# topopt/TopOpt_in_PETSc

Measured on AMD Instinct MI355X. Metric: DOF-updates/s per design iter (assembly+PCG+filter), higher is better.
Workload: dtype f64; 1 GPU; cantilever128: cantilever 128x128x128 elements (6440067 DOF), z-slabs over 1 GPU(s), rmin=2.56h density filter, CG + 5-level GMG (Chebyshev(2)-Jacobi, coarse exact (banded Cholesky + explicit triangular inverse per assembly), Galerkin, cycles per level 1,3,1,1), rtol 1e-05, fine-level eig element bound, cold start, filtered synthetic density seed 12345; n_dof=6440067, levels=5, cycles=1,3,1,1, coarse_solve=direct (2187 rows), cg_its=11, parallelism=zslab1, comm=none, comm_ranks=1, halo_overlap=0

## Files before the change

### include/topopt_amd.h

```cpp
#ifndef TOPOPT_AMD_H
#define TOPOPT_AMD_H

#include <stddef.h>
#include <stdint.h>

#ifdef __cplusplus
extern "C" {
#endif

#define TP_OK 0
#define TP_ERR_ARG 1
#define TP_ERR_STATE 2
#define TP_ERR_DIVERGED 3
#define TP_ERR_COMM 4
#define TP_ERR_HIP 1000

#define TP_MAX_LEVELS 10

typedef struct tp_comm {
    void *user;
    double *send_lo, *send_hi, *recv_lo, *recv_hi;
    double *red;
    long cap;
    int (*exchange)(void *user, long n);
// ... 124 lines not shown
double tp_elasticity_level_lambda(const tp_elasticity *e, int level);
double tp_elasticity_level_lambda_min(const tp_elasticity *e, int level);
int tp_elasticity_coarse_direct_active(const tp_elasticity *e);
int tp_xcd_status(int *giveups, int *xcd_forms_off, int *defer_off);
int tp_elasticity_level_apply(tp_elasticity *e, int level, const double *u, double *y);
int tp_elasticity_level_diag(tp_elasticity *e, int level, double *d);
int tp_elasticity_precond(tp_elasticity *e, const double *r, double *z);
int tp_elasticity_level_pc(tp_elasticity *e, int level, int pc, const double *r, double *z);
int tp_elasticity_level_gmres(tp_elasticity *e, int level, int pc, int m, int its, double rtol, const double *b, double *x,
                              int zero_guess, int *its_done);
int tp_elasticity_smooth(tp_elasticity *e, int level, const double *b, double *x, int k, int zero_guess);
int tp_elasticity_smooth_dot(tp_elasticity *e, int level, const double *b, double *x, int k, int zero_guess, double *dot);
int tp_elasticity_level_residual(tp_elasticity *e, int level, const double *b, const double *x, double *r);
int tp_elasticity_restrict(tp_elasticity *e, int level, const double *rf, double *rc);
int tp_elasticity_prolong_add(tp_elasticity *e, int level, const double *xc, double *xf);
int tp_elasticity_last_stats(const tp_elasticity *e, double *alg_bytes, double *flops, long *kernel_launches);
int tp_elasticity_last_op_form(const tp_elasticity *e, int *form4);

typedef struct tp_filter tp_filter;
int tp_filter_create(tp_filter **f, tp_grid *g, int filterType, double rmin, const tp_solver_opts *pde_opts);
int tp_filter_mult_h(tp_filter *f, const double *x, double *y);
int tp_filter_destroy(tp_filter *f);
int tp_filter_stencil_width(const tp_filter *f);
int tp_filter_last_kernel(const tp_filter *f);
int tp_filter_get_hs(tp_filter *f, double *Hs);
int tp_filter_get_kf(const tp_filter *f, double *kf_host_64);
int tp_filter_project(tp_filter *f, const double *x, double *xTilde, double *xPhys, int projectionFilter, double beta,
                      double eta);
int tp_filter_gradients(tp_filter *f, const double *x, const double *xTilde, double *dfdx, int m, double **dgdx,
                        int projectionFilter, double beta, double eta);
// ... 69 lines not shown
```

### topopt_in_petsc_amd/api.py

```python
import ctypes as C
import os
from dataclasses import dataclass

import torch

from . import lib as _lib
from .comm import SlabComm
from .partition import SlabPartition


class TopOptError(RuntimeError):
    def __init__(self, code, where):
        names = {1: "TP_ERR_ARG", 2: "TP_ERR_STATE", 3: "TP_ERR_DIVERGED", 4: "TP_ERR_COMM"}
        msg = names.get(code, "hipError %d" % (code - 1000) if code >= 1000 else str(code))
        super().__init__("%s failed: %s" % (where, msg))
        self.code = code


def _chk(code, where):
    if code != 0:
        raise TopOptError(code, where)


def check_body_force(b, x_low):
# ... 556 lines not shown

    def level_residual(self, l, b, x):
        r = torch.zeros_like(x)
        _chk(self.L.tp_elasticity_level_residual(self.handle, l, _ptr(b), _ptr(x), _ptr(r)), "tp_elasticity_level_residual")
        return r

    def restrict(self, l, rf):
        rc = self.level_vec(l + 1)
        _chk(self.L.tp_elasticity_restrict(self.handle, l, _ptr(rf), _ptr(rc)), "tp_elasticity_restrict")
        return rc

    def prolong_add(self, l, xc, xf):
        _chk(self.L.tp_elasticity_prolong_add(self.handle, l, _ptr(xc), _ptr(xf)), "tp_elasticity_prolong_add")
        return xf

    def pop_stats(self):
        b, f, n = C.c_double(), C.c_double(), C.c_long()
        self.L.tp_elasticity_last_stats(self.handle, C.byref(b), C.byref(f), C.byref(n))
        return b.value, f.value, n.value

    def last_op_form(self):
        f = (C.c_int * 4)()
        _chk(self.L.tp_elasticity_last_op_form(self.handle, f), "tp_elasticity_last_op_form")
        return tuple(f)


class Filter:

    def __init__(self, grid, filterType, rmin, pde_opts=None):
        self.grid, self.L = grid, grid.L
# ... 282 lines not shown
```

### topopt_in_petsc_amd/csrc/mg.h

```cpp
#pragma once
#include <algorithm>
#include <thread>

#include "galerkin.h"
#include "grid.h"
#include "operators.h"
#include "coarse_run.h"
#include "matfree_tile.h"
#include "fine_tile.h"
#include "fine_u4.h"
#include "coarse_direct.h"
#include "mg_kernels.h"

enum { LV_MATFREE = 0, LV_DIA = 1, LV_MACRO = 2 };

template <int DOF>
struct Level {
    Geom g;
    int kind;
    const double *KE;
    const double *E;
    const uint8_t *mask;
    double *S;
    double *Kel;
// ... 118 lines not shown
        long nown = 0;
        int nb = 0;
        int n_bnd = 0;
        bool out_halo = false;
        bool split = false;
        double bytes = 0.0, flops = 0.0;
    };
    template <int EPI>
    int op(int l, NodeArgs a, bool out_halo = false);
    template <int EPI>
    int op_fine(OpLaunch &c, const NodeArgs &a);
    template <int EPI>
    int op_macro(OpLaunch &c, const NodeArgs &a);
    template <int EPI>
    int op_matfree_node(OpLaunch &c, const NodeArgs &a);
    template <int EPI>
    int op_stencil(OpLaunch &c, const NodeArgs &a);
    static void tile_ranges(const Level<DOF> &L, bool split, int pass, int &lo, int &hi, int &r1lo, int &r1hi);
    int after_boundary(int l, double *out);
    static TileArgs tile_args(const Level<DOF> &L, int lo, int hi, int kz, int r1lo, int r1hi);
    static bool three_term(const Level<DOF> &L) { return DOF == 3 && L.kind == LV_MATFREE && L.use_tile; }
    static int fine_generation(const Level<DOF> &L);
    static bool runs_fine_tile(const Level<DOF> &L) { return fine_generation(L) == 2; }
    int drain_halo(int l);
    int drain_halos();
    template <class F>
    int planes_split(int l, double *out, F launch);
    int halo(int l, double *v);
    int apply(int l, double *u, double *y);
    int apply_krylov(double *u, double *y);
// ... 21 lines not shown
    bool xcd_gaveup();
    void xcd_reset_controls();
    void join_side_streams();
    static int run_rows_per_thread(long rows, int *wgs);
    static int xcd_rows_per_thread(long rows, int *wgs);
    int coarse_run_mode(int l, int nsteps) const;
    bool xcd_eligible(int l, long stage_cap, int max_r) const;
    int coarse_run(int l, const double *b, int it0, int k, double sigma, double delta, int mode);

    int alloc_levels();
    void free_levels();
    int setup_matfree_level(int l, const double *h_KE);
    int gather_owned(Level<DOF> &L, const double *src, Level<DOF> &R, double *dst, int nseg, long src_stride = 0,
                     long dst_stride = 0);
    int setup_replicated();
    int smooth(int l, const double *b, int k, bool zero_guess, int dot_slot = -1, bool first_done = false);
    void cheb_window(int l, double *theta, double *delta) const;
    bool can_fuse_rz() const;
    int vcycle_head(const double *b);
    int vcycle(int l, const double *b, int dot_slot = -1, bool first_done = false, bool zero_guess = true);
    int precond(const double *r, double **z, int dot_slot = -1);
    int solve(const double *b, double *x, int *its_out, double *rnorm_out, double *bnorm_out, double *hist, int hist_cap);
};

#include "mg_op.h"
#include "mg_spectra.h"
#include "mg_coarse.h"
#include "mg_cycle.h"
```

### topopt_in_petsc_amd/csrc/mg_cycle.h

```cpp
#pragma once

template <int DOF>
int MGSolver<DOF>::alloc_levels() {
    for (int l = 0; l < nlv; l++) {
        Level<DOF> &L = lv[l];
        L.g = make_geom(grid, l);
        size_t nb = sizeof(double) * (size_t)L.ndof();
        for (double **p : {&L.b, &L.x, &L.x2, &L.r, &L.d, &L.dinv}) {
            TP_HIP(hipMalloc((void **)p, nb));
            TP_HIP(hipMemsetAsync(*p, 0, nb, grid->stream));
        }
    }
    for (int i = nlv; i < LV_SLOTS; i++) {
        lv[i] = Level<DOF>();
        lv[i].b = lv[i].x = lv[i].x2 = lv[i].r = lv[i].d = lv[i].dinv = lv[i].S = lv[i].Kel = nullptr;
    }
    const bool no_rep = sw_no_replicate();
    replicate = allow_replicate && grid->has_comm && nlv > 1 && !no_rep;
    rep0 = nlv - 1;
    if (replicate) {
        const int from_env = sw_replicate_from();
        if (from_env >= 2 && from_env <= nlv - 1) {
            rep0 = from_env;
            while (rep0 < nlv - 1) {
// ... 142 lines not shown
    if (!replicate) return TP_OK;
    for (int l = rep0; l < nlv; l++) {
        Level<DOF> &L = lv[l], &R = lv[rix(l)];
        if (L.kind != LV_DIA) return TP_ERR_STATE;
        TP_TRY(gather_owned(L, L.S, R, R.S, 27 * DOF, L.ndof(), R.ndof()));
        TP_TRY(gather_owned(L, L.dinv, R, R.dinv, 1));
        if constexpr (DOF == 3) {
            TP_LAUNCH(k_dia_sym_fix, dim3((int)((R.g.owned_nodes() + BLK - 1) / BLK)), dim3(BLK), 0, grid->stream, R.g, R.S, (long)R.ndof());
            count_launch(grid);
        }
    }
    return TP_OK;
}

template <int DOF>
int MGSolver<DOF>::smooth(int l, const double *b, int k, bool zero_guess, int dot_slot, bool first_done) {
    if (replicate && l == nlv - 1) {
        Level<DOF> &R = lv[rix(l)];
        TP_TRY(gather_owned(lv[l], b, R, R.b, 1));
        TP_TRY(smooth(rix(l), R.b, k, zero_guess));
        Level<DOF> &L = lv[l];
        TP_HIP(hipMemcpyAsync(L.x, R.x + (long)DOF * L.g.plane() * L.g.gz0, sizeof(double) * (size_t)L.ndof(),
                              hipMemcpyDeviceToDevice, grid->stream));
        return TP_OK;
    }
    Level<DOF> &L = lv[l];
    if (cd.factored && l == cd.level && dot_slot < 0) return coarse_direct_apply(l, b);
    double theta, delta;
    cheb_window(l, &theta, &delta);
    if (!sg_capturing && dot_slot < 0 && k >= 8 && L.kind == LV_DIA && (L.no_comm || !grid->has_comm) && sw_smooth_graph())
        return smooth_replay(l, b, k, zero_guess, first_done, theta, delta);
// ... 15 lines not shown
    if (it >= 1 && dot_slot < 0) {
        const int mode = coarse_run_mode(l, k - it);
        if (mode) return coarse_run(l, b, it, k, sigma, delta, mode);
    }
    for (; it < k; it++) {
        NodeArgs a{};
        a.x = L.x;
        a.out = L.x2;
        a.b = b;
        a.d = L.d;
        a.dinv = L.dinv;
        a.prev_zero = (zero_guess && it == 1) ? 1 : 0;
        if (it == 0) {
            a.c1 = 0.0;
            a.c2 = 1.0 / theta;
        } else {
            const double rn = 1.0 / (2.0 * sigma - rho);
            a.c1 = rn * rho;
            a.c2 = 2.0 * rn / delta;
            rho = rn;
        }
        TP_TRY(halo(l, L.x));
        if (dot_slot >= 0 && it == k - 1) {
            a.partials = grid->partials;
            a.ticket = tail_ticket(grid);
            a.red_out = grid->scal + dot_slot;
            TP_TRY(op<EPI_CHEB_DOT>(l, a));
        } else {
            TP_TRY(op<EPI_CHEB>(l, a, true));
        }
        std::swap(L.x, L.x2);
    }
    return TP_OK;
}

template <int DOF>
void MGSolver<DOF>::cheb_window(int l, double *theta, double *delta) const {
    const Level<DOF> &L = lv[l];
    const bool solve_level = coarsest(l) && base(l) > 0;
    const double lmin = solve_level ? L.lam_min : opt.cheb_lo * L.lam, lmax = opt.cheb_hi * L.lam;
    *theta = 0.5 * (lmax + lmin);
    *delta = 0.5 * (lmax - lmin);
}

template <int DOF>
bool MGSolver<DOF>::can_fuse_rz() const {
    const int fine_v = sw_fine_v();
    const bool off = sw_no_fuse_rz();
// ... 43 lines not shown
    else TP_TRY(restrict_planes(C.g.own_lo, C.g.own_hi - C.g.own_lo + 1));
    count_launch(grid, 8.0 * DOF * (L.g.owned_nodes() + C.g.owned_nodes()), 2.0 * 27 * DOF * C.g.owned_nodes());
    if (enter_rep) {
        const int r = rix(l + 1);
        Level<DOF> &R = lv[r];
        TP_TRY(gather_owned(C, C.b, R, R.b, 1));
        TP_TRY(vcycle(r, R.b, -1, false));
        for (int c = 1; c < cyc; c++) TP_TRY(vcycle(r, R.b, -1, false, false));
        TP_HIP(hipMemcpyAsync(C.x, R.x + (long)DOF * C.g.plane() * C.g.gz0, sizeof(double) * (size_t)C.ndof(),
                              hipMemcpyDeviceToDevice, grid->stream));
    } else {
        TP_TRY(vcycle(l + 1, C.b, -1, fuse_first));
        for (int c = 1; c < cyc; c++) TP_TRY(vcycle(l + 1, C.b, -1, false, false));
        TP_TRY(halo(l + 1, C.x));
    }
    TP_TRY(planes_split(l, L.x, [&](int p0, int np) -> int {
        const long fpl = L.g.plane();
        TP_LAUNCH((k_prolong_add<DOF>), dim3((int)((fpl * np + BLK - 1) / BLK)), dim3(BLK), 0, grid->stream, C.g, L.g, C.x,
                  L.x, fpl * (p0 - L.g.own_lo), fpl * np);
        return TP_OK;
    }));
    count_launch(grid, 8.0 * DOF * (2 * L.g.owned_nodes() + C.g.owned_nodes()), 2.0 * 8 * DOF * L.g.owned_nodes());
    return smooth(l, b, opt.nsmooth, false, l == 0 ? dot_slot : -1);
}

template <int DOF>
int MGSolver<DOF>::precond(const double *r, double **z, int dot_slot) {
    if (opt.ksp_mode == 1) return refksp_precond(*this, r, z);
    TP_TRY(vcycle(0, r, dot_slot));
    TP_TRY(drain_halos());
// ... 156 lines not shown
```

### topopt_in_petsc_amd/csrc/mg_op.h

```cpp
#pragma once

inline int fine_kz(int planes, int tiles, int fine_v, int SLOTS = 768) {
    if (fine_v >= 2 || fine_v == 0) {
        const int tz1 = SLOTS / tiles;
        if (tz1 >= 1) {
            const int kz1 = (planes + tz1 - 1) / tz1;
            const int n1 = tiles * ((planes + kz1 - 1) / kz1);
            if (kz1 >= 3 && kz1 <= 20 && 10 * n1 >= 9 * SLOTS) return kz1;
        }
    }
    int kz = (int)((long)planes * tiles / 5120);
    kz = kz < 8 ? 8 : (kz > 32 ? 32 : kz);
    if ((long)tiles * ((planes + 7) / 8) < SLOTS) kz = (int)((long)planes * tiles / SLOTS);
    const int kmin = (long)tiles * ((planes + 3) / 4) < 256 ? 2 : 4;
    if (kz < kmin) kz = kmin;
    return kz > planes ? planes : kz;
}

template <int DOF>
int MGSolver<DOF>::fine_generation(const Level<DOF> &L) {
    if (!(DOF == 3 && L.kind == LV_MATFREE && L.use_tile)) return 0;
    const int fine_v = sw_fine_v();
    const int t32 = ((L.g.nx + 30) / 31) * ((L.g.ny + 6) / 7);
    if ((fine_v >= 3 || (fine_v == 0 && t32 >= 160)) && 24.0 * L.g.nodes() < 2.0e9) return 3;
    return (fine_v >= 2 || fine_v == 0) ? 2 : 1;
}

template <int DOF>
template <int EPI>
int MGSolver<DOF>::op(int l, NodeArgs a, bool out_halo) {
    Level<DOF> &L = lv[l];
    OpLaunch c;
    c.l = l;
    c.out_halo = out_halo;
    c.nown = L.g.owned_nodes();
    c.nb = (int)((c.nown + BLK - 1) / BLK);
    last_nblocks = c.nb;
    if (pend[l].ptr && (pend[l].ptr == a.out || pend[l].ptr != a.x)) TP_TRY(drain_halo(l));
    c.n_bnd = (L.g.has_lo ? 1 : 0) + (L.g.has_hi ? 1 : 0);
    const bool tile_level = DOF == 3 && ((L.kind == LV_MATFREE && L.use_tile) || L.kind == LV_MACRO);
    c.split = out_halo && tile_level && EPI != EPI_APPLY_DOT && EPI != EPI_CHEB_DOT && !L.no_comm && c.n_bnd > 0 &&
              halo_can_overlap(grid) && (L.g.own_hi - L.g.own_lo + 1) > c.n_bnd;
    if (DOF == 3 && L.kind == LV_MATFREE && L.use_tile) {
        TP_TRY(op_fine<EPI>(c, a));
    } else if constexpr (EPI == EPI_CHEB_DOT) {
        return TP_ERR_STATE;
    } else if (DOF == 3 && L.kind == LV_MACRO) {
        TP_TRY(op_macro<EPI>(c, a));
    } else if (L.kind == LV_MATFREE) {
        TP_TRY(op_matfree_node<EPI>(c, a));
    } else {
        TP_TRY(op_stencil<EPI>(c, a));
    }
    double bytes = c.bytes;
    if (EPI == EPI_RESID) bytes += 8.0 * DOF * c.nown;
    if (EPI == EPI_CHEB || EPI == EPI_CHEB_DOT) bytes += (three_term(L) ? ((a.c1 != 0.0 && !a.prev_zero) ? 2.0 : 1.0) : 4.0) * 8.0 * DOF * c.nown;
    if (grid->kt_on && l == 0 && (EPI == EPI_CHEB || EPI == EPI_CHEB_DOT) && !c.split && !sg_capturing) grid->kt_bytes += bytes;
    count_launch(grid, bytes, c.flops);
    if (c.split) grid->launches++;
    return TP_OK;
}

template <int DOF>
void MGSolver<DOF>::tile_ranges(const Level<DOF> &L, bool split, int pass, int &lo, int &hi, int &r1lo, int &r1hi) {
    lo = L.g.own_lo, hi = L.g.own_hi, r1lo = 0, r1hi = -1;
    if (!split) return;
    if (pass == 0) {
        if (L.g.has_lo && L.g.has_hi) lo = hi = L.g.own_lo, r1lo = r1hi = L.g.own_hi;
        else if (L.g.has_lo) hi = lo;
        else lo = hi;
    } else {
// ... 137 lines not shown
            c.flops = 2.0 * 27 * (double)c.nown;
            as_stencil = true;
        }
    }
    if (!as_stencil) {
        MatfreeOp<DOF> o{L.KE, L.E, L.mask, L.g};
        TP_LAUNCH((k_node<DOF, MatfreeOp<DOF>, EPI>), dim3(c.nb), dim3(BLK), 0, grid->stream, o, a);
        c.bytes = 16.0 * DOF * c.nown + (L.E ? 8.0 * L.g.own_elems() : 0.0);
        c.flops = 2.0 * (8 * DOF) * (8 * DOF) * (double)L.g.own_elems();
    }
    last_form[0] = 3, last_form[1] = as_stencil ? 1 : 0, last_form[2] = last_form[3] = 0;
    return TP_OK;
}

template <int DOF>
template <int EPI>
int MGSolver<DOF>::op_stencil(OpLaunch &c, const NodeArgs &a) {
    Level<DOF> &L = lv[c.l];
    DiaOp<DOF> o{L.S, L.ndof(), L.g};
    const long rows_all = c.nown * DOF;
    const int nbr_all = (int)((rows_all + BLK - 1) / BLK);
    const int split_env = sw_dia_split();
    const bool by_node = sw_dia_node();
    const int rsplit = split_env >= 0 ? split_env : (nbr_all < 128 ? 9 : ((DOF == 3 && by_node) ? 3 : (nbr_all < 512 ? 3 : 1)));
    const bool sym = !sw_no_dia_sym();
    auto launch_rows = [&](long t0, long tn, long t1, long tn1) -> int {
        o.t0 = t0, o.tn = tn, o.t1 = t1, o.tn1 = tn1;
        const long rows = tn < 0 ? rows_all : tn + tn1;
        int nbr = 0;
        if (rsplit == 9) {
            nbr = (int)((rows + BLK / 9 - 1) / (BLK / 9));
            TP_LAUNCH((k_dia_row_split<DOF, EPI, 9>), dim3(nbr), dim3(BLK), 0, grid->stream, o, a);
            last_form[0] = 4, last_form[1] = 9, last_form[2] = 0, last_form[3] = 0;
        } else if (rsplit == 3) {
            bool done = false;
            if constexpr (DOF == 3) {
                if (by_node && EPI != EPI_APPLY_DOT) {
                    nbr = (int)((rows / 3 + 63) / 64);
                    if (sym) {
                        TP_LAUNCH((k_dia_node3<EPI, true>), dim3(nbr), dim3(192), 0, grid->stream, o, a);
                        last_form[0] = 4, last_form[1] = 3, last_form[2] = 1, last_form[3] = 1;
                    } else {
                        TP_LAUNCH((k_dia_node3<EPI, false>), dim3(nbr), dim3(192), 0, grid->stream, o, a);
                        last_form[0] = 4, last_form[1] = 3, last_form[2] = 1, last_form[3] = 0;
                    }
                    done = true;
                }
            }
            if (!done) {
                nbr = (int)((rows + BLK / 3 - 1) / (BLK / 3));
                if (sym) {
                    TP_LAUNCH((k_dia_row_split<DOF, EPI, 3, true>), dim3(nbr), dim3(BLK), 0, grid->stream, o, a);
                    last_form[0] = 4, last_form[1] = 3, last_form[2] = 0, last_form[3] = 1;
                } else {
                    TP_LAUNCH((k_dia_row_split<DOF, EPI, 3>), dim3(nbr), dim3(BLK), 0, grid->stream, o, a);
                    last_form[0] = 4, last_form[1] = 3, last_form[2] = 0, last_form[3] = 0;
                }
            }
        } else {
            nbr = (int)((rows + BLK - 1) / BLK);
// ... 86 lines not shown
```

### topopt_in_petsc_amd/csrc/operators.h

```cpp
#pragma once
#include "common.h"

template <int DOF>
struct MatfreeOp {
    const double *__restrict__ KE;
    const double *__restrict__ E;
    const uint8_t *__restrict__ mask;
    Geom g;

    __device__ inline void load_masked(const double *__restrict__ u, long nb, double ub[DOF]) const {
#pragma unroll
        for (int c = 0; c < DOF; c++) ub[c] = u[nb * DOF + c];
        if (mask) {
            const unsigned m = mask[nb];
#pragma unroll
            for (int c = 0; c < DOF; c++)
                if ((m >> c) & 1u) ub[c] = 0.0;
        }
    }

    __device__ inline void apply(const double *__restrict__ u, int i, int j, int k, long n, double y[DOF]) const {
        constexpr int ED = 8 * DOF;
#pragma unroll
        for (int r = 0; r < DOF; r++) y[r] = 0.0;
// ... 137 lines not shown
struct NodeArgs {
    const double *x;
    double *out;
    const double *b;
    double *d;
    const double *dinv;
    double c1, c2;
    int prev_zero;
    double *partials;
    unsigned *ticket;
    double *red_out;
    const double *pz;
    double *pnew;
    const double *pscal;
    int slot_new, slot_old;
};

template <int DOF, class Op, int EPI>
__global__ __launch_bounds__(BLK) void k_node(Op op, NodeArgs a) {
    const Geom &g = op.g;
    const long plane = g.plane();
    const long t = blockIdx.x * (long)BLK + threadIdx.x;
    double pdot = 0.0;
    if (t < g.owned_nodes()) {
        const int k = g.own_lo + (int)(t / plane);
        const int rem = (int)(t % plane);
        const int j = rem / g.nx, i = rem % g.nx;
        const long n = t + plane * g.own_lo;
        double y[DOF];
        op.apply(a.x, i, j, k, n, y);
// ... 156 lines not shown
    double s[DOF];
#pragma unroll
    for (int r = 0; r < DOF; r++) s[r] = 0.0;
    for (int kk = 0; kk <= mk; kk++)
        for (int jj = 0; jj <= mj; jj++)
            for (int ii = 0; ii <= mi; ii++) {
                const double w = (mi ? 0.5 : 1.0) * (mj ? 0.5 : 1.0) * (mk ? 0.5 : 1.0);
                const long nc = (long)(I0 + ii) + (long)gc.nx * ((J0 + jj) + (long)gc.ny * (K0 + kk));
#pragma unroll
                for (int r = 0; r < DOF; r++) s[r] = fma(w, xc[nc * DOF + r], s[r]);
            }
#pragma unroll
    for (int r = 0; r < DOF; r++) xf[nf * DOF + r] += s[r];
}

__device__ inline double cheb_dn(double c1, double d, double c2, double dinv, double b, double y) {
#pragma clang fp contract(off)
    const double t = c2 * (dinv * (b - y));
    return fma(c1, d, t);
}

template <int DOF, int EPI>
__global__ __launch_bounds__(BLK) void k_dia_row(DiaOp<DOF> op, NodeArgs a) {
    const Geom &g = op.g;
    const long plane = g.plane();
    const long tl = blockIdx.x * (long)BLK + threadIdx.x;
    double pdot = 0.0;
    if (tl < op.rows_here()) {
        const long t = op.row_of(tl);
        const long q = t + plane * g.own_lo * DOF;
// ... 52 lines not shown
        const bool ok = k + dk >= 0 && k + dk < g.nzl && j + dj >= 0 && j + dj < g.ny && i + di >= 0 && i + di < g.nx;
        if (!(ok && k + dk >= g.own_lo && k + dk <= g.own_hi)) continue;
        const long nb = n + di + (long)g.nx * (dj + (long)g.ny * dk);
#pragma unroll
        for (int r = 0; r < 3; r++)
#pragma unroll
            for (int c = 0; c < 3; c++)
                acc[r][c] += S[(long)(blk * 3 + c) * nrows + n * 3 + r] - S[(long)((26 - blk) * 3 + r) * nrows + nb * 3 + c];
    }
#pragma unroll
    for (int r = 0; r < 3; r++)
#pragma unroll
        for (int c = 0; c < 3; c++) S[(long)(81 + c) * nrows + n * 3 + r] = acc[r][c];
}

template <int EPI, bool SYM>
__global__ __launch_bounds__(192) void k_dia_node3(DiaOp<3> op, NodeArgs a) {
    constexpr int SPLIT = 3;
    constexpr int NPB = 64;
    typedef double d2u __attribute__((ext_vector_type(2), aligned(8)));
    __shared__ double s_part[SPLIT == 3 ? 3 : 1][3][SPLIT == 3 ? NPB : 1];
    const Geom &g = op.g;
    const long plane = g.plane();
    const int part = SPLIT == 3 ? __builtin_amdgcn_readfirstlane(threadIdx.x >> 6) : 0, r = SPLIT == 3 ? (threadIdx.x & 63) : threadIdx.x;
    const int nbk = gridDim.x, x8 = blockIdx.x & 7;
    const int bid = SYM ? x8 * (nbk >> 3) + min(x8, nbk & 7) + (blockIdx.x >> 3) : blockIdx.x;
    const long tl = ((long)bid * NPB + r) * 3;
    const bool valid = tl < op.rows_here();
    const long q0 = (valid ? op.row_of(tl) : 0) + plane * g.own_lo * 3;
    const long n = q0 / 3;
    const double *__restrict__ u = a.x;
    const double *__restrict__ S = op.S;
    double e_b[3] = {0, 0, 0}, e_d[3] = {0, 0, 0}, e_di[3] = {0, 0, 0}, e_u[3] = {0, 0, 0};
    if (valid && part == 0) {
#pragma unroll
        for (int rr = 0; rr < 3; rr++) {
            if (EPI == EPI_RESID || EPI == EPI_CHEB) e_b[rr] = a.b[q0 + rr];
            if (EPI == EPI_CHEB) e_d[rr] = a.d[q0 + rr], e_di[rr] = a.dinv[q0 + rr];
            if (EPI == EPI_APPLY && a.dinv) e_di[rr] = a.dinv[q0 + rr];
            if (EPI == EPI_CHEB || EPI == EPI_APPLY_DOT || SYM) e_u[rr] = u[q0 + rr];
        }
    }
    double e_ds[3][3] = {{0, 0, 0}, {0, 0, 0}, {0, 0, 0}};
    if (SYM && valid && part == 0) {
#pragma unroll
        for (int c = 0; c < 3; c++)
#pragma unroll
            for (int rr = 0; rr < 3; rr++) e_ds[rr][c] = S[(long)(81 + c) * op.nrows + q0 + rr];
    }
    double y[3] = {0.0, 0.0, 0.0};
    if (valid) {
        const int k = (int)(n / plane);
        const int rem = (int)(n % plane);
        const int j = rem / g.nx, i = rem % g.nx;
#pragma unroll
        for (int dkk = 0; dkk < (SPLIT == 3 ? 1 : 3); dkk++) {
            const int dk = (SPLIT == 3 ? part : dkk) - 1;
            const bool okk = k + dk >= 0 && k + dk < g.nzl;
            const bool own_k = k + dk >= g.own_lo && k + dk <= g.own_hi;
#pragma unroll
            for (int dj = -1; dj <= 1; dj++) {
                const bool okj = okk && j + dj >= 0 && j + dj < g.ny;
#pragma unroll
                for (int di = -1; di <= 1; di++) {
                    const bool ok = okj && i + di >= 0 && i + di < g.nx;
                    const int blk = (dk + 1) * 9 + (dj + 1) * 3 + (di + 1);
                    const long nb = ok ? n + di + (long)g.nx * (dj + (long)g.ny * dk) : n;
                    const bool mir = SYM && blk > 13 && ok && own_k;
                    const double *__restrict__ un = u + nb * 3;
                    const d2u u01 = *(const d2u *)un;
                    const double uv[3] = {u01.x, u01.y, un[2]};
                    double T[3][3];
#pragma unroll
                    for (int kq = 0; kq < 3; kq++) {
                        const long ad = mir ? (long)((26 - blk) * 3 + kq) * op.nrows + nb * 3 : (long)(blk * 3 + kq) * op.nrows + q0;
                        const d2u t01 = *(const d2u *)(S + ad);
                        T[kq][0] = t01.x;
                        T[kq][1] = t01.y;
                        T[kq][2] = S[ad + 2];
                    }
#pragma unroll
                    for (int c = 0; c < 3; c++)
#pragma unroll
                        for (int rr = 0; rr < 3; rr++) {
                            const double cf = (rr == c) ? T[c][c] : (mir ? T[rr][c] : T[c][rr]);
                            y[rr] = fma(cf, uv[c], y[rr]);
// ... 30 lines not shown
                const double dn = cheb_dn(a.c1, e_d[rr], a.c2, e_di[rr], e_b[rr], yy);
                a.d[q] = dn;
                a.out[q] = e_u[rr] + dn;
            } else {
                a.out[q] = yy;
                pdot = fma(e_u[rr], yy, pdot);
            }
        }
    }
    if (EPI == EPI_APPLY_DOT) {
        const double v[1] = {block_sum(pdot)};
        reduce_tail<1>(v, a.partials, gridDim.x, blockIdx.x, a.ticket, a.red_out);
    }
}

template <int DOF, int EPI, int SPLIT, bool SYM = false>
__global__ __launch_bounds__(BLK) void k_dia_row_split(DiaOp<DOF> op, NodeArgs a) {
    constexpr int RPB = BLK / SPLIT;
    __shared__ double s_part[SPLIT][RPB];
    const Geom &g = op.g;
    const long plane = g.plane();
    const int part = threadIdx.x / RPB, r = threadIdx.x % RPB;
    const int nbk = gridDim.x, x8 = blockIdx.x & 7;
    const int bid = SYM ? x8 * (nbk >> 3) + min(x8, nbk & 7) + (blockIdx.x >> 3) : blockIdx.x;
    const long tl = bid * (long)RPB + r;
    const bool valid = part < SPLIT && tl < op.rows_here();
    const long t = valid ? op.row_of(tl) : 0;
    const long q = t + plane * g.own_lo * DOF;
    const double *__restrict__ u = a.x;
    double e_b = 0.0, e_d = 0.0, e_di = 0.0, e_u = 0.0;
    if (valid && part == 0) {
        if (EPI == EPI_RESID || EPI == EPI_CHEB) e_b = a.b[q];
        if (EPI == EPI_CHEB) e_d = a.d[q], e_di = a.dinv[q];
        if (EPI == EPI_APPLY && a.dinv) e_di = a.dinv[q];
        if (EPI == EPI_CHEB || EPI == EPI_APPLY_DOT) e_u = u[q];
    }
    double e_ds[DOF], e_un[DOF];
#pragma unroll
    for (int c = 0; c < DOF; c++) e_ds[c] = 0.0, e_un[c] = 0.0;
    if (SYM && DOF == 3 && valid && part == 0) {
        const long nn = q / DOF;
#pragma unroll
        for (int c = 0; c < DOF; c++) {
            e_ds[c] = op.S[(long)(27 * DOF + c) * op.nrows + q];
            e_un[c] = u[nn * DOF + c];
        }
    }
    if (valid) {
        const long n = q / DOF;
        const int k = (int)(n / plane);
        const int rem = (int)(n % plane);
        const int j = rem / g.nx, i = rem % g.nx;
        double y = 0.0;
        const int dk = (SPLIT == 3 ? part : part / 3) - 1;
        const bool okk = k + dk >= 0 && k + dk < g.nzl;
#pragma unroll
        for (int djj = 0; djj < (SPLIT == 9 ? 1 : 3); djj++) {
            const int dj = (SPLIT == 9 ? part % 3 : djj) - 1;
            const bool okj = okk && j + dj >= 0 && j + dj < g.ny;
#pragma unroll
            for (int di = -1; di <= 1; di++) {
                const bool ok = okj && i + di >= 0 && i + di < g.nx;
                const int blk = (dk + 1) * 9 + (dj + 1) * 3 + (di + 1);
                const long nb = ok ? n + di + (long)g.nx * (dj + (long)g.ny * dk) : n;
                const bool mir = SYM && blk > 13 && ok && k + dk >= g.own_lo && k + dk <= g.own_hi;
                const int rr = (int)(q - n * DOF);
#pragma unroll
                for (int c = 0; c < DOF; c++) {
                    const long ad = mir ? (long)((26 - blk) * DOF + rr) * op.nrows + nb * DOF + c
                                        : (long)(blk * DOF + c) * op.nrows + q;
                    y = fma(op.S[ad], u[nb * DOF + c], y);
                }
            }
        }
        s_part[part][r] = y;
    }
    __syncthreads();
    double pdot = 0.0;
    if (valid && part == 0) {
        double y = s_part[0][r];
#pragma unroll
// ... 24 lines not shown
```

### topopt_in_petsc_amd/csrc/switches.h

```cpp
#pragma once
#include <cstdlib>
#include <cstring>

inline bool &tp_xcd_disabled() {
    static bool off = false;
    return off;
}
inline bool &tp_defer_disabled() {
    static bool off = false;
    return off;
}
inline int &tp_giveup_count() {
    static int n = 0;
    return n;
}

inline bool sw_set(const char *name) { return getenv(name) != nullptr; }
inline int sw_int(const char *name, int dflt) { return getenv(name) ? atoi(getenv(name)) : dflt; }
inline bool sw_not_zero(const char *name) { return !(getenv(name) && atoi(getenv(name)) == 0); }


inline bool tp_debug_sync() {
    static const bool v = getenv("TP_DEBUG_SYNC") != nullptr && atoi(getenv("TP_DEBUG_SYNC")) != 0;
    return v;
// ... 104 lines not shown

inline bool sw_no_replicate() {
    static const bool v = sw_set("TP_NO_REPLICATE");
    return v;
}
inline int sw_replicate_from() {
    static const int v = (getenv("TP_REPLICATE_FROM") && *getenv("TP_REPLICATE_FROM")) ? atoi(getenv("TP_REPLICATE_FROM")) : -1;
    return v;
}
inline bool sw_no_fuse_rz() {
    static const bool v = sw_set("TP_NO_FUSE_RZ");
    return v;
}
inline bool sw_no_fuse_first() {
    static const bool v = sw_set("TP_NO_FUSE_FIRST");
    return v;
}
inline bool sw_no_spec_head() {
    static const bool v = sw_set("TP_NO_SPEC_HEAD");
    return v;
}
inline bool sw_no_cg_fuse() {
    static const bool v = sw_set("TP_NO_CG_FUSE");
    return v;
}
inline bool sw_cg_nt() {
    static const bool v = sw_not_zero("TP_CG_NT");
    return v;
}

// ... 57 lines not shown
```

### topopt_in_petsc_amd/csrc/topopt_amd.hip

```cpp
#include <string>

#include "elements.h"
#include "mg.h"
#include "refksp.h"
#include "rccl_comm.h"

extern "C" int tp_grid_create(tp_grid **out, const tp_grid_opts *o) {
    if (!out || !o) return TP_ERR_ARG;
    if (o->nx < 2 || o->ny < 2 || o->nz < 2 || o->nranks < 1 || o->rank < 0 || o->rank >= o->nranks) return TP_ERR_ARG;
    if ((o->nz - 1) % o->nranks) return TP_ERR_ARG;
    if (o->nranks > 1 && !o->comm) return TP_ERR_ARG;
    TP_HIP(hipSetDevice(o->device));
    tp_grid *g = new tp_grid();
    g->o = *o;
    g->stream = (hipStream_t)o->stream;
    g->has_comm = o->nranks > 1;
    if (g->has_comm) {
        g->comm = g->comm_host = *o->comm;
        const bool want = sw_overlap();
        if (want && hipStreamCreateWithFlags(&g->comm_stream, hipStreamNonBlocking) == hipSuccess &&
            hipEventCreateWithFlags(&g->ev_ready, hipEventDisableTiming) == hipSuccess)
            g->overlap = true;
        else
            (void)hipGetLastError();
// ... 1253 lines not shown
    if (l < 0 || l + 1 >= mg.nlv) return TP_ERR_ARG;
    TP_TRY(mg.halo(l, const_cast<double *>(rf)));
    const Geom &C = mg.lv[l + 1].g;
    TP_LAUNCH((k_restrict<3>), dim3((int)((C.owned_nodes() + BLK - 1) / BLK)), dim3(BLK), 0,
                       e->grid->stream, C, mg.lv[l].g, rf, rc);
    return TP_OK;
}
extern "C" int tp_elasticity_prolong_add(tp_elasticity *e, int l, const double *xc, double *xf) {
    MGSolver<3> &mg = e->mg;
    if (l < 0 || l + 1 >= mg.nlv) return TP_ERR_ARG;
    TP_TRY(mg.halo(l + 1, const_cast<double *>(xc)));
    TP_LAUNCH((k_prolong_add<3>), dim3((int)((mg.lv[l].g.owned_nodes() + BLK - 1) / BLK)), dim3(BLK), 0,
                       e->grid->stream, mg.lv[l + 1].g, mg.lv[l].g, xc, xf);
    return TP_OK;
}
extern "C" int tp_elasticity_last_stats(const tp_elasticity *e, double *alg_bytes, double *flops, long *launches) {
    if (alg_bytes) *alg_bytes = e->grid->alg_bytes;
    if (flops) *flops = e->grid->flops;
    if (launches) *launches = e->grid->launches;
    e->grid->alg_bytes = e->grid->flops = 0.0;
    e->grid->launches = 0;
    return TP_OK;
}
extern "C" int tp_elasticity_last_op_form(const tp_elasticity *e, int *form4) {
    if (!e || !form4) return TP_ERR_ARG;
    for (int i = 0; i < 4; i++) form4[i] = e->mg.last_form[i];
    return TP_OK;
}

#include "response.h"
// ... 11 lines not shown
```

### topopt_in_petsc_amd/lib.py

```python
import ctypes as C
import os
import subprocess

_HERE = os.path.dirname(os.path.abspath(__file__))
SO_PATH = os.environ.get("TP_LIB") or os.path.join(_HERE, "libtopopt_amd.so")
_LIB = None


class LibraryMissing(RuntimeError):
    pass


def build(force=False):
    src = os.path.join(_HERE, "csrc")
    deps = [os.path.join(src, f) for f in os.listdir(src)] + [os.path.join(_HERE, "..", "include", "topopt_amd.h")]
    if force or not os.path.exists(SO_PATH) or any(os.path.getmtime(d) > os.path.getmtime(SO_PATH) for d in deps):
        subprocess.check_call(["make", "-C", src], stdout=subprocess.DEVNULL)
    return SO_PATH


class GridOpts(C.Structure):
    _fields_ = [("nx", C.c_int), ("ny", C.c_int), ("nz", C.c_int), ("hx", C.c_double), ("hy", C.c_double),
                ("hz", C.c_double), ("rank", C.c_int), ("nranks", C.c_int), ("device", C.c_int),
                ("stream", C.c_void_p), ("comm", C.c_void_p)]
# ... 85 lines not shown
    "tp_elasticity_level_lambda": (_d, [_vp, _i]),
    "tp_elasticity_level_lambda_min": (_d, [_vp, _i]),
    "tp_elasticity_coarse_direct_active": (_i, [_vp]),
    "tp_xcd_status": (_i, [C.POINTER(_i), C.POINTER(_i), C.POINTER(_i)]),
    "tp_elasticity_level_apply": (_i, [_vp, _i, _vp, _vp]),
    "tp_elasticity_level_diag": (_i, [_vp, _i, _vp]),
    "tp_elasticity_set_cycles": (_i, [_vp, _vp, _i]),
    "tp_elasticity_precond": (_i, [_vp, _vp, _vp]),
    "tp_elasticity_level_pc": (_i, [_vp, _i, _i, _vp, _vp]),
    "tp_elasticity_level_gmres": (_i, [_vp, _i, _i, _i, _i, _d, _vp, _vp, _i, C.POINTER(_i)]),
    "tp_elasticity_smooth": (_i, [_vp, _i, _vp, _vp, _i, _i]),
    "tp_elasticity_smooth_dot": (_i, [_vp, _i, _vp, _vp, _i, _i, C.POINTER(C.c_double)]),
    "tp_elasticity_level_residual": (_i, [_vp, _i, _vp, _vp, _vp]),
    "tp_elasticity_restrict": (_i, [_vp, _i, _vp, _vp]),
    "tp_elasticity_prolong_add": (_i, [_vp, _i, _vp, _vp]),
    "tp_elasticity_last_stats": (_i, [_vp, C.POINTER(_d), C.POINTER(_d), C.POINTER(_l)]),
    "tp_elasticity_last_op_form": (_i, [_vp, C.POINTER(_i)]),
    "tp_filter_create": (_i, [C.POINTER(_vp), _vp, _i, _d, C.POINTER(SolverOpts)]),
    "tp_filter_destroy": (_i, [_vp]),
    "tp_filter_stencil_width": (_i, [_vp]),
    "tp_filter_last_kernel": (_i, [_vp]),
    "tp_filter_get_hs": (_i, [_vp, _vp]),
    "tp_filter_get_kf": (_i, [_vp, _vp]),
    "tp_filter_project": (_i, [_vp, _vp, _vp, _vp, _i, _d, _d]),
    "tp_filter_gradients": (_i, [_vp, _vp, _vp, _vp, _i, C.POINTER(_vp), _i, _d, _d]),
    "tp_filter_mnd": (_i, [_vp, _vp, C.POINTER(_d)]),
    "tp_filter_last_pde_its": (_i, [_vp, C.POINTER(_i), C.POINTER(_d)]),
    "tp_pdefilter_elem_to_node": (_i, [_vp, _vp, _vp]),
    "tp_pdefilter_solve": (_i, [_vp, _vp, _vp]),
    "tp_pdefilter_node_to_elem": (_i, [_vp, _vp, _vp]),
# ... 70 lines not shown
```

Measured before the change: 542.1 million DOF-updates/s.

## Fuse coarse-grid prolongation into the first post-smoothing Chebyshev stencil step

On assembled-stencil (DIA) levels, the trilinear prolongation of the coarse correction is folded into the first Chebyshev iteration of post-smoothing. It is not run as a separate k_prolong_add kernel. The row-split and node3 stencil kernels stage u+P·xc for the needed plane neighbourhood in shared memory, so neither the fine vector nor the prolonged correction is written and re-read. This saves one launch and a full fine-vector read-modify-write per fused level. In exchange, each staged node recomputes the interpolation, there are extra shared-memory syncs, and the fusion only applies on single-rank, non-graph paths for coarse DIA levels.

After: 540.5 million DOF-updates/s. Within noise of the previous version (-0.3%).

```diff
diff --git a/include/topopt_amd.h b/include/topopt_amd.h
--- a/include/topopt_amd.h
+++ b/include/topopt_amd.h
@@ -162,6 +162,7 @@
 int tp_elasticity_level_residual(tp_elasticity *e, int level, const double *b, const double *x, double *r);
 int tp_elasticity_restrict(tp_elasticity *e, int level, const double *rf, double *rc);
 int tp_elasticity_prolong_add(tp_elasticity *e, int level, const double *xc, double *xf);
+int tp_elasticity_prolong_smooth(tp_elasticity *e, int level, const double *xc, const double *b, double *x, int k);
 int tp_elasticity_last_stats(const tp_elasticity *e, double *alg_bytes, double *flops, long *kernel_launches);
 int tp_elasticity_last_op_form(const tp_elasticity *e, int *form4);
 
diff --git a/topopt_in_petsc_amd/api.py b/topopt_in_petsc_amd/api.py
--- a/topopt_in_petsc_amd/api.py
+++ b/topopt_in_petsc_amd/api.py
@@ -594,6 +594,10 @@
         _chk(self.L.tp_elasticity_prolong_add(self.handle, l, _ptr(xc), _ptr(xf)), "tp_elasticity_prolong_add")
         return xf
 
+    def prolong_smooth(self, l, xc, b, x, k):
+        _chk(self.L.tp_elasticity_prolong_smooth(self.handle, l, _ptr(xc), _ptr(b), _ptr(x), k), "tp_elasticity_prolong_smooth")
+        return x
+
     def pop_stats(self):
         b, f, n = C.c_double(), C.c_double(), C.c_long()
         self.L.tp_elasticity_last_stats(self.handle, C.byref(b), C.byref(f), C.byref(n))
diff --git a/topopt_in_petsc_amd/csrc/mg.h b/topopt_in_petsc_amd/csrc/mg.h
--- a/topopt_in_petsc_amd/csrc/mg.h
+++ b/topopt_in_petsc_amd/csrc/mg.h
@@ -156,6 +156,8 @@
     int op_macro(OpLaunch &c, const NodeArgs &a);
     template <int EPI>
     int op_matfree_node(OpLaunch &c, const NodeArgs &a);
+    int stencil_split(const Level<DOF> &L) const;
+    int prolong_form(const Level<DOF> &L) const;
     template <int EPI>
     int op_stencil(OpLaunch &c, const NodeArgs &a);
     static void tile_ranges(const Level<DOF> &L, bool split, int pass, int &lo, int &hi, int &r1lo, int &r1hi);
@@ -207,7 +209,8 @@
     int gather_owned(Level<DOF> &L, const double *src, Level<DOF> &R, double *dst, int nseg, long src_stride = 0,
                      long dst_stride = 0);
     int setup_replicated();
-    int smooth(int l, const double *b, int k, bool zero_guess, int dot_slot = -1, bool first_done = false);
+    int smooth(int l, const double *b, int k, bool zero_guess, int dot_slot = -1, bool first_done = false, const double *corr = nullptr);
+    bool fuse_prolong_ok(int l, int k) const;
     void cheb_window(int l, double *theta, double *delta) const;
     bool can_fuse_rz() const;
     int vcycle_head(const double *b);
diff --git a/topopt_in_petsc_amd/csrc/mg_cycle.h b/topopt_in_petsc_amd/csrc/mg_cycle.h
--- a/topopt_in_petsc_amd/csrc/mg_cycle.h
+++ b/topopt_in_petsc_amd/csrc/mg_cycle.h
@@ -180,7 +180,8 @@
 }
 
 template <int DOF>
-int MGSolver<DOF>::smooth(int l, const double *b, int k, bool zero_guess, int dot_slot, bool first_done) {
+int MGSolver<DOF>::smooth(int l, const double *b, int k, bool zero_guess, int dot_slot, bool first_done, const double *corr) {
+    if (corr && !(fuse_prolong_ok(l, k) && !zero_guess && dot_slot < 0)) return TP_ERR_STATE;
     if (replicate && l == nlv - 1) {
         Level<DOF> &R = lv[rix(l)];
         TP_TRY(gather_owned(lv[l], b, R, R.b, 1));
@@ -226,6 +227,7 @@
         if (it == 0) {
             a.c1 = 0.0;
             a.c2 = 1.0 / theta;
+            if (corr) a.pe = corr, a.peg = lv[l + 1].g;
         } else {
             const double rn = 1.0 / (2.0 * sigma - rho);
             a.c1 = rn * rho;
@@ -244,6 +246,14 @@
         std::swap(L.x, L.x2);
     }
     return TP_OK;
+}
+
+template <int DOF>
+bool MGSolver<DOF>::fuse_prolong_ok(int l, int k) const {
+    if (DOF != 3 || sw_no_fuse_prolong() || grid->has_comm || opt.ksp_mode != 0 || sg_capturing) return false;
+    if (l < 0 || l + 1 >= nlv || k < 1) return false;
+    if (k >= 8 && sw_smooth_graph()) return false;
+    return prolong_form(lv[l]) != 0;
 }
 
 template <int DOF>
@@ -317,6 +327,7 @@
         for (int c = 1; c < cyc; c++) TP_TRY(vcycle(l + 1, C.b, -1, false, false));
         TP_TRY(halo(l + 1, C.x));
     }
+    if (fuse_prolong_ok(l, opt.nsmooth)) return smooth(l, b, opt.nsmooth, false, -1, false, C.x);
     TP_TRY(planes_split(l, L.x, [&](int p0, int np) -> int {
         const long fpl = L.g.plane();
         TP_LAUNCH((k_prolong_add<DOF>), dim3((int)((fpl * np + BLK - 1) / BLK)), dim3(BLK), 0, grid->stream, C.g, L.g, C.x,
diff --git a/topopt_in_petsc_amd/csrc/mg_op.h b/topopt_in_petsc_amd/csrc/mg_op.h
--- a/topopt_in_petsc_amd/csrc/mg_op.h
+++ b/topopt_in_petsc_amd/csrc/mg_op.h
@@ -37,6 +37,7 @@
     c.nb = (int)((c.nown + BLK - 1) / BLK);
     last_nblocks = c.nb;
     if (pend[l].ptr && (pend[l].ptr == a.out || pend[l].ptr != a.x)) TP_TRY(drain_halo(l));
+    if (a.pe && !(EPI == EPI_CHEB && !grid->has_comm && prolong_form(L))) return TP_ERR_STATE;
     c.n_bnd = (L.g.has_lo ? 1 : 0) + (L.g.has_hi ? 1 : 0);
     const bool tile_level = DOF == 3 && ((L.kind == LV_MATFREE && L.use_tile) || L.kind == LV_MACRO);
     c.split = out_halo && tile_level && EPI != EPI_APPLY_DOT && EPI != EPI_CHEB_DOT && !L.no_comm && c.n_bnd > 0 &&
@@ -55,6 +56,7 @@
     double bytes = c.bytes;
     if (EPI == EPI_RESID) bytes += 8.0 * DOF * c.nown;
     if (EPI == EPI_CHEB || EPI == EPI_CHEB_DOT) bytes += (three_term(L) ? ((a.c1 != 0.0 && !a.prev_zero) ? 2.0 : 1.0) : 4.0) * 8.0 * DOF * c.nown;
+    if (a.pe) bytes += 8.0 * DOF * a.peg.nodes();
     if (grid->kt_on && l == 0 && (EPI == EPI_CHEB || EPI == EPI_CHEB_DOT) && !c.split && !sg_capturing) grid->kt_bytes += bytes;
     count_launch(grid, bytes, c.flops);
     if (c.split) grid->launches++;
@@ -222,15 +224,28 @@
 }
 
 template <int DOF>
+int MGSolver<DOF>::stencil_split(const Level<DOF> &L) const {
+    const int nbr_all = (int)((L.g.owned_nodes() * DOF + BLK - 1) / BLK);
+    const int split_env = sw_dia_split();
+    return split_env >= 0 ? split_env : (nbr_all < 128 ? 9 : ((DOF == 3 && sw_dia_node()) ? 3 : (nbr_all < 512 ? 3 : 1)));
+}
+
+template <int DOF>
+int MGSolver<DOF>::prolong_form(const Level<DOF> &L) const {
+    if (DOF != 3 || L.kind != LV_DIA) return 0;
+    const int rsplit = stencil_split(L);
+    if (rsplit == 9) return 9;
+    return (rsplit == 3 && sw_dia_node() && L.g.nx <= NODE3_PE_NX) ? 3 : 0;
+}
+
+template <int DOF>
 template <int EPI>
 int MGSolver<DOF>::op_stencil(OpLaunch &c, const NodeArgs &a) {
     Level<DOF> &L = lv[c.l];
     DiaOp<DOF> o{L.S, L.ndof(), L.g};
     const long rows_all = c.nown * DOF;
-    const int nbr_all = (int)((rows_all + BLK - 1) / BLK);
-    const int split_env = sw_dia_split();
     const bool by_node = sw_dia_node();
-    const int rsplit = split_env >= 0 ? split_env : (nbr_all < 128 ? 9 : ((DOF == 3 && by_node) ? 3 : (nbr_all < 512 ? 3 : 1)));
+    const int rsplit = stencil_split(L);
     const bool sym = !sw_no_dia_sym();
     auto launch_rows = [&](long t0, long tn, long t1, long tn1) -> int {
         o.t0 = t0, o.tn = tn, o.t1 = t1, o.tn1 = tn1;
@@ -238,20 +253,26 @@
         int nbr = 0;
         if (rsplit == 9) {
             nbr = (int)((rows + BLK / 9 - 1) / (BLK / 9));
-            TP_LAUNCH((k_dia_row_split<DOF, EPI, 9>), dim3(nbr), dim3(BLK), 0, grid->stream, o, a);
+            bool done = false;
+            if constexpr (DOF == 3 && EPI == EPI_CHEB) {
+                if (a.pe) {
+                    TP_LAUNCH((k_dia_row_split<3, EPI_CHEB, 9, false, true>), dim3(nbr), dim3(BLK), 0, grid->stream, o, a);
+                    done = true;
+                }
+            }
+            if (!done) TP_LAUNCH((k_dia_row_split<DOF, EPI, 9>), dim3(nbr), dim3(BLK), 0, grid->stream, o, a);
             last_form[0] = 4, last_form[1] = 9, last_form[2] = 0, last_form[3] = 0;
         } else if (rsplit == 3) {
             bool done = false;
             if constexpr (DOF == 3) {
                 if (by_node && EPI != EPI_APPLY_DOT) {
                     nbr = (int)((rows / 3 + 63) / 64);
-                    if (sym) {
-                        TP_LAUNCH((k_dia_node3<EPI, true>), dim3(nbr), dim3(192), 0, grid->stream, o, a);
-                        last_form[0] = 4, last_form[1] = 3, last_form[2] = 1, last_form[3] = 1;
-                    } else {
-                        TP_LAUNCH((k_dia_node3<EPI, false>), dim3(nbr), dim3(192), 0, grid->stream, o, a);
-                        last_form[0] = 4, last_form[1] = 3, last_form[2] = 1, last_form[3] = 0;
-                    }
+                    constexpr bool CHEB = EPI == EPI_CHEB;
+                    if (CHEB && a.pe && sym) TP_LAUNCH((k_dia_node3<EPI, true, CHEB>), dim3(nbr), dim3(192), 0, grid->stream, o, a);
+                    else if (CHEB && a.pe) TP_LAUNCH((k_dia_node3<EPI, false, CHEB>), dim3(nbr), dim3(192), 0, grid->stream, o, a);
+                    else if (sym) TP_LAUNCH((k_dia_node3<EPI, true>), dim3(nbr), dim3(192), 0, grid->stream, o, a);
+                    else TP_LAUNCH((k_dia_node3<EPI, false>), dim3(nbr), dim3(192), 0, grid->stream, o, a);
+                    last_form[0] = 4, last_form[1] = 3, last_form[2] = 1, last_form[3] = sym ? 1 : 0;
                     done = true;
                 }
             }
diff --git a/topopt_in_petsc_amd/csrc/operators.h b/topopt_in_petsc_amd/csrc/operators.h
--- a/topopt_in_petsc_amd/csrc/operators.h
+++ b/topopt_in_petsc_amd/csrc/operators.h
@@ -175,6 +175,8 @@
     double *pnew;
     const double *pscal;
     int slot_new, slot_old;
+    const double *pe;
+    Geom peg;
 };
 
 template <int DOF, class Op, int EPI>
@@ -361,6 +363,28 @@
     for (int r = 0; r < DOF; r++) xf[nf * DOF + r] += s[r];
 }
 
+__device__ inline void prolonged3(const Geom &gc, const double *__restrict__ xc, int i, int j, int k, double s[3]) {
+    const int I0 = i >> 1, J0 = j >> 1, K0 = k >> 1;
+    const int mi = i & 1, mj = j & 1, mk = k & 1;
+    typedef double d2u __attribute__((ext_vector_type(2), aligned(8)));
+    double v[8][3];
+#pragma unroll
+    for (int q = 0; q < 8; q++) {
+        const int ii = q & 1 & mi, jj = (q >> 1) & 1 & mj, kk = (q >> 2) & mk;
+        const long nc = (long)(I0 + ii) + (long)gc.nx * ((J0 + jj) + (long)gc.ny * (K0 + kk));
+        const d2u v01 = *(const d2u *)(xc + nc * 3);
+        v[q][0] = v01.x, v[q][1] = v01.y, v[q][2] = xc[nc * 3 + 2];
+    }
+    const double w = (mi ? 0.5 : 1.0) * (mj ? 0.5 : 1.0) * (mk ? 0.5 : 1.0);
+    s[0] = s[1] = s[2] = 0.0;
+#pragma unroll
+    for (int q = 0; q < 8; q++) {
+        const bool present = (q & 1) <= mi && ((q >> 1) & 1) <= mj && (q >> 2) <= mk;
+#pragma unroll
+        for (int r = 0; r < 3; r++) s[r] = present ? fma(w, v[q][r], s[r]) : s[r];
+    }
+}
+
 __device__ inline double cheb_dn(double c1, double d, double c2, double dinv, double b, double y) {
 #pragma clang fp contract(off)
     const double t = c2 * (dinv * (b - y));
@@ -443,12 +467,16 @@
         for (int c = 0; c < 3; c++) S[(long)(81 + c) * nrows + n * 3 + r] = acc[r][c];
 }
 
-template <int EPI, bool SYM>
+constexpr int NODE3_PE_NX = 65;
+template <int EPI, bool SYM, bool PE = false>
 __global__ __launch_bounds__(192) void k_dia_node3(DiaOp<3> op, NodeArgs a) {
+    static_assert(!PE || EPI == EPI_CHEB, "the prolonged input exists for the Chebyshev step");
     constexpr int SPLIT = 3;
     constexpr int NPB = 64;
+    constexpr int SEG = NPB + 2 * NODE3_PE_NX + 2;
     typedef double d2u __attribute__((ext_vector_type(2), aligned(8)));
     __shared__ double s_part[SPLIT == 3 ? 3 : 1][3][SPLIT == 3 ? NPB : 1];
+    __shared__ double s_x[PE ? 3 : 1][3][PE ? SEG : 1];
     const Geom &g = op.g;
     const long plane = g.plane();
     const int part = SPLIT == 3 ? __builtin_amdgcn_readfirstlane(threadIdx.x >> 6) : 0, r = SPLIT == 3 ? (threadIdx.x & 63) : threadIdx.x;
@@ -467,7 +495,7 @@
             if (EPI == EPI_RESID || EPI == EPI_CHEB) e_b[rr] = a.b[q0 + rr];
             if (EPI == EPI_CHEB) e_d[rr] = a.d[q0 + rr], e_di[rr] = a.dinv[q0 + rr];
             if (EPI == EPI_APPLY && a.dinv) e_di[rr] = a.dinv[q0 + rr];
-            if (EPI == EPI_CHEB || EPI == EPI_APPLY_DOT || SYM) e_u[rr] = u[q0 + rr];
+            if ((EPI == EPI_CHEB || EPI == EPI_APPLY_DOT || SYM) && !PE) e_u[rr] = u[q0 + rr];
         }
     }
     double e_ds[3][3] = {{0, 0, 0}, {0, 0, 0}, {0, 0, 0}};
@@ -476,6 +504,26 @@
         for (int c = 0; c < 3; c++)
 #pragma unroll
             for (int rr = 0; rr < 3; rr++) e_ds[rr][c] = S[(long)(81 + c) * op.nrows + q0 + rr];
+    }
+    if constexpr (PE) {
+        const long first = (long)bid * NPB - g.nx - 1, nn = g.nodes();
+        const int seglen = NPB + 2 * g.nx + 2;
+        for (int t = threadIdx.x; t < 3 * seglen; t += 192) {
+            const int sg = t / seglen, o = t - sg * seglen;
+            const long m = first + (sg - 1) * plane + o;
+            if (m >= 0 && m < nn) {
+                const int mk = (int)(m / plane), mrem = (int)(m % plane);
+                double pe[3];
+                prolonged3(a.peg, a.pe, mrem % g.nx, mrem / g.nx, mk, pe);
+#pragma unroll
+                for (int c = 0; c < 3; c++) s_x[sg][c][o] = u[m * 3 + c] + pe[c];
+            }
+        }
+        __syncthreads();
+        if (valid && part == 0) {
+#pragma unroll
+            for (int rr = 0; rr < 3; rr++) e_u[rr] = s_x[1][rr][r + g.nx + 1];
+        }
     }
     double y[3] = {0.0, 0.0, 0.0};
     if (valid) {
@@ -496,9 +544,16 @@
                     const int blk = (dk + 1) * 9 + (dj + 1) * 3 + (di + 1);
                     const long nb = ok ? n + di + (long)g.nx * (dj + (long)g.ny * dk) : n;
                     const bool mir = SYM && blk > 13 && ok && own_k;
-                    const double *__restrict__ un = u + nb * 3;
-                    const d2u u01 = *(const d2u *)un;
-                    const double uv[3] = {u01.x, u01.y, un[2]};
+                    double uv[3];
+                    if constexpr (PE) {
+                        const int sg = ok ? part : 1, o = r + g.nx + 1 + (ok ? dj * g.nx + di : 0);
+#pragma unroll
+                        for (int c = 0; c < 3; c++) uv[c] = s_x[sg][c][o];
+                    } else {
+                        const double *__restrict__ un = u + nb * 3;
+                        const d2u u01 = *(const d2u *)un;
+                        uv[0] = u01.x, uv[1] = u01.y, uv[2] = un[2];
+                    }
                     double T[3][3];
 #pragma unroll
                     for (int kq = 0; kq < 3; kq++) {
@@ -559,10 +614,13 @@
     }
 }
 
-template <int DOF, int EPI, int SPLIT, bool SYM = false>
+template <int DOF, int EPI, int SPLIT, bool SYM = false, bool PE = false>
 __global__ __launch_bounds__(BLK) void k_dia_row_split(DiaOp<DOF> op, NodeArgs a) {
+    static_assert(!PE || (DOF == 3 && EPI == EPI_CHEB && SPLIT == 9 && !SYM), "the prolonged input exists for the 9-way Chebyshev step");
     constexpr int RPB = BLK / SPLIT;
     __shared__ double s_part[SPLIT][RPB];
+    constexpr int RUN = RPB / 3 + 3;
+    __shared__ double s_x[PE ? 9 : 1][3][PE ? RUN : 1];
     const Geom &g = op.g;
     const long plane = g.plane();
     const int part = threadIdx.x / RPB, r = threadIdx.x % RPB;
@@ -578,7 +636,7 @@
         if (EPI == EPI_RESID || EPI == EPI_CHEB) e_b = a.b[q];
         if (EPI == EPI_CHEB) e_d = a.d[q], e_di = a.dinv[q];
         if (EPI == EPI_APPLY && a.dinv) e_di = a.dinv[q];
-        if (EPI == EPI_CHEB || EPI == EPI_APPLY_DOT) e_u = u[q];
+        if ((EPI == EPI_CHEB && !PE) || EPI == EPI_APPLY_DOT) e_u = u[q];
     }
     double e_ds[DOF], e_un[DOF];
 #pragma unroll
@@ -590,6 +648,31 @@
             e_ds[c] = op.S[(long)(27 * DOF + c) * op.nrows + q];
             e_un[c] = u[nn * DOF + c];
         }
+    }
+    double cf[PE ? 3 : 1][PE ? 3 : 1];
+    const long nfirst = PE ? (bid * (long)RPB) / 3 : 0;
+    if constexpr (PE) {
+        if (valid) {
+#pragma unroll
+            for (int di = 0; di < 3; di++)
+#pragma unroll
+                for (int c = 0; c < 3; c++) cf[di][c] = op.S[(long)((part * 3 + di) * 3 + c) * op.nrows + q];
+        }
+        const long nrows = op.rows_here(), qlast = min(bid * (long)RPB + RPB, nrows) - 1, nn = g.nodes();
+        const int run = (int)(qlast / 3 - nfirst) + 3;
+        if ((int)threadIdx.x < 9 * RUN) {
+            const int p = threadIdx.x / RUN, o = threadIdx.x % RUN;
+            const long m = nfirst - 1 + o + (p / 3 - 1) * plane + (p % 3 - 1) * g.nx;
+            if (o < run && m >= 0 && m < nn) {
+                const int mk = (int)(m / plane), mrem = (int)(m % plane);
+                double pe[3];
+                prolonged3(a.peg, a.pe, mrem % g.nx, mrem / g.nx, mk, pe);
+#pragma unroll
+                for (int c = 0; c < 3; c++) s_x[p][c][o] = u[m * 3 + c] + pe[c];
+            }
+        }
+        __syncthreads();
+        if (valid && part == 0) e_u = s_x[4][q % 3][q / 3 - nfirst + 1];
     }
     if (valid) {
         const long n = q / DOF;
@@ -610,6 +693,12 @@
                 const long nb = ok ? n + di + (long)g.nx * (dj + (long)g.ny * dk) : n;
                 const bool mir = SYM && blk > 13 && ok && k + dk >= g.own_lo && k + dk <= g.own_hi;
                 const int rr = (int)(q - n * DOF);
+                if constexpr (PE) {
+                    const int o = (int)(n - nfirst) + 1 + (ok ? di : 0);
+#pragma unroll
+                    for (int c = 0; c < 3; c++) y = fma(cf[di + 1][c], s_x[ok ? part : 4][c][o], y);
+                    continue;
+                }
 #pragma unroll
                 for (int c = 0; c < DOF; c++) {
                     const long ad = mir ? (long)((26 - blk) * DOF + rr) * op.nrows + nb * DOF + c
diff --git a/topopt_in_petsc_amd/csrc/switches.h b/topopt_in_petsc_amd/csrc/switches.h
--- a/topopt_in_petsc_amd/csrc/switches.h
+++ b/topopt_in_petsc_amd/csrc/switches.h
@@ -142,6 +142,10 @@
 }
 inline bool sw_no_fuse_first() {
     static const bool v = sw_set("TP_NO_FUSE_FIRST");
+    return v;
+}
+inline bool sw_no_fuse_prolong() {
+    static const bool v = sw_set("TP_NO_FUSE_PROLONG");
     return v;
 }
 inline bool sw_no_spec_head() {
diff --git a/topopt_in_petsc_amd/csrc/topopt_amd.hip b/topopt_in_petsc_amd/csrc/topopt_amd.hip
--- a/topopt_in_petsc_amd/csrc/topopt_amd.hip
+++ b/topopt_in_petsc_amd/csrc/topopt_amd.hip
@@ -1291,6 +1291,25 @@
                        e->grid->stream, mg.lv[l + 1].g, mg.lv[l].g, xc, xf);
     return TP_OK;
 }
+extern "C" int tp_elasticity_prolong_smooth(tp_elasticity *e, int l, const double *xc, const double *b, double *x, int k) {
+    if (!e || !e->assembled) return TP_ERR_STATE;
+    MGSolver<3> &mg = e->mg;
+    if (l < 0 || l + 1 >= mg.nlv || !xc || !b || !x || k < 1) return TP_ERR_ARG;
+    Level<3> &L = mg.lv[l];
+    const size_t nb = sizeof(double) * (size_t)L.ndof();
+    TP_HIP(hipMemcpyAsync(L.x, x, nb, hipMemcpyDeviceToDevice, e->grid->stream));
+    TP_TRY(mg.halo(l + 1, const_cast<double *>(xc)));
+    if (mg.fuse_prolong_ok(l, k)) {
+        TP_TRY(mg.smooth(l, b, k, false, -1, false, xc));
+    } else {
+        TP_LAUNCH((k_prolong_add<3>), dim3((int)((L.g.owned_nodes() + BLK - 1) / BLK)), dim3(BLK), 0, e->grid->stream, mg.lv[l + 1].g, L.g, xc, L.x);
+        count_launch(e->grid);
+        TP_TRY(mg.smooth(l, b, k, false));
+    }
+    TP_TRY(mg.drain_halos());
+    TP_HIP(hipMemcpyAsync(x, L.x, nb, hipMemcpyDeviceToDevice, e->grid->stream));
+    return TP_OK;
+}
 extern "C" int tp_elasticity_last_stats(const tp_elasticity *e, double *alg_bytes, double *flops, long *launches) {
     if (alg_bytes) *alg_bytes = e->grid->alg_bytes;
     if (flops) *flops = e->grid->flops;
diff --git a/topopt_in_petsc_amd/lib.py b/topopt_in_petsc_amd/lib.py
--- a/topopt_in_petsc_amd/lib.py
+++ b/topopt_in_petsc_amd/lib.py
@@ -123,6 +123,7 @@
     "tp_elasticity_level_residual": (_i, [_vp, _i, _vp, _vp, _vp]),
     "tp_elasticity_restrict": (_i, [_vp, _i, _vp, _vp]),
     "tp_elasticity_prolong_add": (_i, [_vp, _i, _vp, _vp]),
+    "tp_elasticity_prolong_smooth": (_i, [_vp, _i, _vp, _vp, _vp, _i]),
     "tp_elasticity_last_stats": (_i, [_vp, C.POINTER(_d), C.POINTER(_d), C.POINTER(_l)]),
     "tp_elasticity_last_op_form": (_i, [_vp, C.POINTER(_i)]),
     "tp_filter_create": (_i, [C.POINTER(_vp), _vp, _i, _d, C.POINTER(SolverOpts)]),
```
